# mhnazeri/PMoE

Measured on AMD Instinct MI355X. Metric: samples/sec fwd+bwd, 256x256 RGB 4-expert PMoE, higher is better.
Workload: dtype bf16; 1 GPU; 4-expert MoE (PMoE experts), 256x256x3 x4 frames, batch 64/GPU, fwd+moe_loss+bwd, dropout 0.3; global_batch=64, parallelism=dp1

## Files before the change

### pmoe_amd/csrc/conv_wgrad.hip

```cpp
#include "conv_common.h"
#include <stdlib.h>
#include "kernels.h"

template <typename T> struct WgradCfg;
template <> struct WgradCfg<bf16> { static constexpr int WCO = 2, WCI = 2, WK = 2, NW = 8; };
template <> struct WgradCfg<float> { static constexpr int WCO = 1, WCI = 1, WK = 4, NW = 4; };

typedef __attribute__((address_space(3))) s16x4 lds_s16x4;

__device__ __forceinline__ s16x4 tr_read(const char* p) {
    return __builtin_amdgcn_ds_read_tr16_b64_v4i16((lds_s16x4*)(p));
}

template <typename T, int TAPS, int MAXV>
__global__ void __launch_bounds__(WgradCfg<T>::NW * 64) conv_wgrad_kernel(const WgradArgs a) {
    constexpr int NTHR = WgradCfg<T>::NW * 64;
    constexpr int LOG_RB = 7, RB = 128;
    constexpr int VE = 16 / (int)sizeof(T);
    constexpr int CKW = RB / (int)sizeof(T);
    constexpr int WCI = WgradCfg<T>::WCI, WK = WgradCfg<T>::WK;
    constexpr int KS = TAPS == 9 ? 3 : 1;
    constexpr int MAXDY = 256 * 8 / NTHR;
    extern __shared__ __attribute__((aligned(16))) char smem[];

// ... 91 lines not shown
                int pA[2], ppB[2];
#pragma unroll
                for (int tt = 0; tt < 2; ++tt) {
                    const int p = p0 + 8 * (g >> 1) + 4 * tt + q;
                    pA[tt] = p;
                    const int mx = p & (TW - 1), my = (p >> lTW) & (TH - 1), pn = p >> (lTW + lTH);
                    ppB[tt] = (pn * PH + my * S) * PW + mx * S;
                }
                const int ca = (co_sub * 32 + cblk) * 2, cb = (ci_sub * 32 + cblk) * 2;
                bf16x8 fa;
#pragma unroll
                for (int tt = 0; tt < 2; ++tt) {
                    const s16x4 r = tr_read(dyt + pA[tt] * RS + ca);
                    const bf16x4 rb = __builtin_bit_cast(bf16x4, r);
#pragma unroll
                    for (int i = 0; i < 4; ++i) fa[4 * tt + i] = rb[i];
                }
                const char* bB[2] = {patch + ppB[0] * RS + cb, patch + ppB[1] * RS + cb};
#pragma unroll
                for (int tap = 0; tap < TAPS; ++tap) {
                    const int tapoff = ((tap / KS) * PW + (tap % KS)) * RS;
                    bf16x8 fb;
#pragma unroll
                    for (int tt = 0; tt < 2; ++tt) {
                        const s16x4 r = tr_read(bB[tt] + tapoff);
                        const bf16x4 rb = __builtin_bit_cast(bf16x4, r);
#pragma unroll
                        for (int i = 0; i < 4; ++i) fb[4 * tt + i] = rb[i];
                    }
                    acc[tap] = __builtin_amdgcn_mfma_f32_32x32x16_bf16(fa, fb, acc[tap], 0, 0, 0);
                }
            } else {
#pragma unroll
                for (int m = 0; m < 8; ++m) {
                    const int p = p0 + 2 * m + h;
                    const int mx = p & (TW - 1), my = (p >> lTW) & (TH - 1), pn = p >> (lTW + lTH);
                    const int ppb = (pn * PH + my * S) * PW + mx * S;
                    const float av = *reinterpret_cast<const float*>(dyt + p * RS + (l31 << 2));
#pragma unroll
                    for (int tap = 0; tap < TAPS; ++tap) {
                        const int pp = ppb + (tap / KS) * PW + (tap % KS);
                        const float bv = *reinterpret_cast<const float*>(patch + pp * RS + (l31 << 2));
                        acc[tap] = __builtin_amdgcn_mfma_f32_32x32x2f32(av, bv, acc[tap], 0, 0, 0);
                    }
                }
            }
        }
    }

    constexpr int TPR = TAPS == 9 ? 3 : 1;
    constexpr int TILE_WAVES = WCO * WCI;
    float* red = reinterpret_cast<float*>(smem);
    const int tw = wave % TILE_WAVES;
    const int cin = ci0 + ci_sub * 32 + l31;
    const size_t slab = a.per_image ? (size_t)e * a.ipe + split
                                    : (size_t)split * gridDim.z + e;
    float* dst = (a.per_image || nsplit == 1) ? a.dw : a.part;
#pragma unroll
    for (int t0 = 0; t0 < TAPS; t0 += TPR) {
        __syncthreads();
        if (k_sub > 0) {
#pragma unroll
            for (int tp = 0; tp < TPR; ++tp)
#pragma unroll
                for (int r = 0; r < 16; ++r)
                    red[((((k_sub - 1) * TPR + tp) * TILE_WAVES + tw) * 16 + r) * 64 + lane] = acc[t0 + tp][r];
        }
        __syncthreads();
        if (k_sub == 0) {
#pragma unroll
            for (int tp = 0; tp < TPR; ++tp) {
                float* base = dst + ((slab * TAPS + t0 + tp) * a.CoutP) * a.CinP;
#pragma unroll
                for (int r = 0; r < 16; ++r) {
                    float v = acc[t0 + tp][r];
#pragma unroll
                    for (int k = 1; k < WK; ++k) v += red[((((k - 1) * TPR + tp) * TILE_WAVES + tw) * 16 + r) * 64 + lane];
                    const int cout = co0 + co_sub * 32 + (r & 3) + 8 * (r >> 2) + 4 * h;
                    base[(size_t)cout * a.CinP + cin] = v;
                }
            }
        }
    }
}

template <int PIN, int WCI = 2, bool PAIRS = false, int REQ = 0>
__global__ void __launch_bounds__(512) conv_wgrad_dma_kernel(const WgradArgs a, const int magic_pw, const int magic_ph) {
    constexpr int TAPS = 9, RS = 128, CKW = 64;
    static_assert(!PAIRS || WCI == 1, "tap pairs: the narrow wave layout only");
    static_assert(REQ == 0 || (WCI == 2 && !PAIRS && PIN == 1), "precomputed requests: the 2 x 2 x 2 wave layout only");
    constexpr int WCO = 2, WK = 8 / (WCI * WCO);
    typedef __attribute__((address_space(3))) void lds_void;
    extern __shared__ __attribute__((aligned(16))) char smem[];

    const int tid = threadIdx.x, lane = tid & 63;
    const int wave = __builtin_amdgcn_readfirstlane(tid >> 6);
    const int l31 = lane & 31, h = lane >> 5;
    const int ci_sub = wave % WCI, co_sub = (wave / WCI) % WCO, k_sub = wave / (WCI * WCO);

    const int e = blockIdx.z;
    const int n_ci_blk = (a.Cin + CKW - 1) / CKW;
    const int npairs = n_ci_blk * ((a.Cout + CKW - 1) / CKW);
    const unsigned flat = xcd_remap(blockIdx.x, gridDim.x);
    const int nsplit = (int)(gridDim.x / npairs);
    const int pair = (int)(flat % npairs), split = (int)(flat / npairs);
    const int cob = pair / n_ci_blk, cib = pair % n_ci_blk;
    const int co0 = cob * CKW, ci0 = cib * CKW;

    const int lTW = a.lTW, lTH = a.lTH;
    const int TW = 1 << lTW, TH = 1 << lTH;
    const int PW = TW + 2, PH = TH + 2;
    const int NPIX = a.TN * PH * PW;
    const int NPIECE = (NPIX + 7) >> 3;
    const int BMP = a.TN << (lTW + lTH);
    const int XB = NPIECE << 10;
    const int pair_bytes = (BMP << 7) + XB;
    const int my_pieces = (NPIECE - wave + 7) >> 3;

    f32x16 acc[TAPS];
#pragma unroll
    for (int t = 0; t < TAPS; ++t)
#pragma unroll
        for (int k = 0; k < 16; ++k) acc[t][k] = 0.f;

    const int mbpe = a.n_groups * a.tiles_y * a.tiles_x;
    const int mb_begin = split * a.mb_per_wg;
    int mb_end = mb_begin + a.mb_per_wg;
    if (mb_end > mbpe) mb_end = mbpe;

    const bf16* xb = (const bf16*)a.x + (a.x_shared ? (size_t)0 : (size_t)e * a.ipe * a.H * a.W * a.x_ld) + a.x_coff + ci0;
    const bf16* dyb = (const bf16*)a.dy + (size_t)e * a.ipe * a.Ho * a.Wo * a.dy_ld + a.dy_coff + co0;
    const __amdgpu_buffer_rsrc_t rs_x = __builtin_amdgcn_make_buffer_rsrc(
        (void*)xb, (short)0, (int)(((long long)a.ipe * a.H * a.W * a.x_ld - a.x_coff - ci0) * 2), 0x00020000);
    const __amdgpu_buffer_rsrc_t rs_dy = __builtin_amdgcn_make_buffer_rsrc(
        (void*)dyb, (short)0, (int)(((long long)a.ipe * a.Ho * a.Wo * a.dy_ld - a.dy_coff - co0) * 2), 0x00020000);
    constexpr int OOB = 0x7ff80000;

    auto issue = [&](int mbi, int buf) {
        int t = mbi;
        const int px_t = t % a.tiles_x; t /= a.tiles_x;
        const int py_t = t % a.tiles_y; t /= a.tiles_y;
        const int n0 = t * a.TN;
        const int oy0 = py_t * TH, ox0 = px_t * TW;
        char* base = smem + buf * pair_bytes;
#pragma unroll
        for (int i = 0; i < 4; ++i) {
            const int p = ((wave + 8 * i) << 3) + (lane >> 3);
            const int mx = p & (TW - 1), my = (p >> lTW) & (TH - 1), pn = p >> (lTW + lTH);
            const int n = n0 + pn, oy = oy0 + my, ox = ox0 + mx;
            const int j = (lane & 7) ^ (((p >> 1) & 1) << 2);
            const bool ok = n < a.ipe && oy < a.Ho && ox < a.Wo && co0 + j * 8 < a.Cout;
            const int voff = ok ? ((((n * a.Ho + oy) * a.Wo + ox) * a.dy_ld) << 1) + (j << 4) : OOB;
            __builtin_amdgcn_raw_ptr_buffer_load_lds(rs_dy, (lds_void*)(base + ((wave + 8 * i) << 10)), 16, voff, 0, 0, 0);
        }
#pragma unroll
        for (int i = 0; i < 6; ++i) {
            if (i < my_pieces) {
                const int pp = ((wave + 8 * i) << 3) + (lane >> 3);
                const int rowq = (pp * magic_pw) >> 16, px = pp - rowq * PW;
                const int pn = (rowq * magic_ph) >> 16, prow = rowq - pn * PH;
                const int n = n0 + pn, Y = oy0 - a.pad + prow, X = ox0 - a.pad + px;
                const int j = (lane & 7) ^ (((px >> 1) & 1) << 2);
                const bool ok = pp < NPIX && n < a.ipe && (unsigned)Y < (unsigned)a.H && (unsigned)X < (unsigned)a.W &&
                                ci0 + j * 8 < a.Cin;
                const int voff = ok ? ((((n * a.H + Y) * a.W + X) * a.x_ld) << 1) + (j << 4) : OOB;
                __builtin_amdgcn_raw_ptr_buffer_load_lds(rs_x, (lds_void*)(base + (BMP << 7) + ((wave + 8 * i) << 10)), 16,
// ... 688 lines not shown
    const int pipe_unset = INT_MIN, pipe_sw = sw("PMOE_WGRAD_PIPE", pipe_unset);
    const bool narrow = a.Cin <= 32 && sw("PMOE_WGRAD_NARROW", 1);
    const bool v2 = !narrow && sw("PMOE_WGRAD_V2", 1) && pipe_sw == pipe_unset && (a.lTW == 4 || a.lTW == 5) && a.ipe <= 511;
    p->kind = v2 ? WGRAD_DMA2 : WGRAD_DMA;
    p->code = narrow ? 7109 : v2 ? 7309 : 7009;
    p->grid = dim3(p->nsplit * tiles, 1, p->E); p->block = dim3(512);
    p->smem = sm < 49152 ? 49152 : sm;
    const int pipe = pipe_sw == pipe_unset ? 1 : pipe_sw;
    p->pin = 1; p->wci = narrow ? 1 : 2;
    if (v2) {
#ifdef PMOE_STAMP
    } else if (pipe == 2 || pipe == 3) {
        p->pin = pipe; p->wci = 2;
#endif
    } else if (narrow) {
        p->pairs = a.Cin <= 16;
        if (p->smem < (size_t)3 * 3 * 2 * 4096) p->smem = (size_t)3 * 3 * 2 * 4096;
    } else if (pipe == 0) {
        p->pin = 0;
    } else {
        const int req = a.ipe > 511 ? 0 : sw("PMOE_WGRAD_REQ", 1);
        p->req = req == 1 || req == 2 ? req : 0;
    }
    return true;
}

template <typename T> constexpr int wgrad_fold_waves = (WgradCfg<T>::WK - 1) * WgradCfg<T>::WCO * WgradCfg<T>::WCI;

int wgrad_select(const WgradArgs& a0, int dtype, const WgradBn& bn, WgradPlan* p) {
    *p = WgradPlan{};
    p->a = a0;
    WgradArgs& a = p->a;
    auto done = [p](int code) { return p->code = code; };
    if (bn.fused) return done(wgrad_bnbwd_plan(dtype, bn.z_ld, p));
    if (dtype != PMOE_DT_BF16 && dtype != PMOE_DT_F32) return done(PMOE_ERR_ARG);
    const int esz = p->esz = dtype == PMOE_DT_BF16 ? 2 : 4;
    const int CKW = 128 / esz, VEh = 16 / esz, NW = esz == 2 ? WgradCfg<bf16>::NW : WgradCfg<float>::NW;
    const int M1 = 48 / NW, M2 = 80 / NW;
    if (a.Cin % VEh || a.Cout % VEh || a.CinP < a.Cin || a.CoutP < a.Cout) return done(PMOE_ERR_ARG);
    if (a.CinP != (a.Cin + CKW - 1) / CKW * CKW || a.CoutP != (a.Cout + CKW - 1) / CKW * CKW) return done(PMOE_ERR_ARG);
    if ((a.ks != 1 && a.ks != 3) || (a.stride != 1 && a.stride != 2) || a.N % a.ipe) return done(PMOE_ERR_ARG);
    p->E = a.N / a.ipe; p->taps = a.ks * a.ks;
    const int lstride = a.ks == 1 ? 1 : a.stride;
    int lBM = 8, PW, PH, NPIX, need;
    size_t smem;
    for (;; --lBM) {
        if (lBM < 6) return done(PMOE_ERR_UNSUPPORTED);
        set_tile(a, pixel_tile(a.Ho, a.Wo, a.ipe, lBM, 5));
        PW = patch_extent(a.lTW, a.ks, lstride); PH = patch_extent(a.lTH, a.ks, lstride);
        NPIX = a.TN * PH * PW;
        need = (NPIX * 8 + NW * 64 - 1) / (NW * 64);
        smem = ((size_t)(1 << lBM) + NPIX) * 192;
        if (need <= M2 && smem <= 150 * 1024) break;
    }
    const int mbpe = a.n_groups * a.tiles_y * a.tiles_x;
    const int tiles = ((a.Cout + CKW - 1) / CKW) * ((a.Cin + CKW - 1) / CKW);
    const int target = 256;
    int want = (target + tiles * p->E - 1) / (tiles * p->E);
    if (want < 1) want = 1;
    if (want > mbpe) want = mbpe;
    a.mb_per_wg = (mbpe + want - 1) / want;
    if (a.per_image) {
        if (a.TN != 1) return done(PMOE_ERR_UNSUPPORTED);
        a.mb_per_wg = a.tiles_y * a.tiles_x;
    }
    a.slice_fastest = 0;
    p->nsplit = (mbpe + a.mb_per_wg - 1) / a.mb_per_wg;
    p->ws_floats = (a.per_image || p->nsplit == 1) ? 0 : (long long)p->nsplit * p->E * p->taps * a.CoutP * a.CinP;
    if (esz == 2 && lBM == 8 && wgrad_dma_plan(NPIX, PW, PH, tiles, p)) return p->code;
    p->kind = WGRAD_TILE;
    p->maxv = need <= M1 ? M1 : M2;
    p->grid = dim3(p->nsplit * tiles, 1, p->E); p->block = dim3(NW * 64);
    const size_t fold = (size_t)(esz == 2 ? wgrad_fold_waves<bf16> : wgrad_fold_waves<float>) * (p->taps == 9 ? 3 : 1) * 4096;
    p->smem = smem < fold ? fold : smem;
    return p->code = 6000 + p->taps * 100 + p->maxv;
}

template <auto KERNEL, typename... Args> static int wgrad_go(const WgradPlan& p, hipStream_t st, const Args&... args) {
    return launch<KERNEL>(p.grid, p.block, p.smem, st, p.a, args...);
}

template <typename T> static int wgrad_tile_launch(const WgradPlan& p, hipStream_t st) {
    constexpr int M1 = 48 / WgradCfg<T>::NW, M2 = 80 / WgradCfg<T>::NW;
    if (p.maxv == M1) return p.taps == 9 ? wgrad_go<conv_wgrad_kernel<T, 9, M1>>(p, st) : wgrad_go<conv_wgrad_kernel<T, 1, M1>>(p, st);
    return p.taps == 9 ? wgrad_go<conv_wgrad_kernel<T, 9, M2>>(p, st) : wgrad_go<conv_wgrad_kernel<T, 1, M2>>(p, st);
}

static int wgrad_dma_launch(const WgradPlan& p, hipStream_t st) {
    switch (p.pin) {
    case 0: return wgrad_go<conv_wgrad_dma_kernel<0>>(p, st, p.mpw, p.mph);
#ifdef PMOE_STAMP
    case 2: return wgrad_go<conv_wgrad_dma_kernel<2>>(p, st, p.mpw, p.mph);
    case 3: return wgrad_go<conv_wgrad_dma_kernel<3>>(p, st, p.mpw, p.mph);
#endif
    }
    if (p.wci == 1 && p.pairs) return wgrad_go<conv_wgrad_dma_kernel<1, 1, true>>(p, st, p.mpw, p.mph);
    if (p.wci == 1) return wgrad_go<conv_wgrad_dma_kernel<1, 1>>(p, st, p.mpw, p.mph);
    if (p.req == 2) return wgrad_go<conv_wgrad_dma_kernel<1, 2, false, 2>>(p, st, p.mpw, p.mph);
    if (p.req == 1) return wgrad_go<conv_wgrad_dma_kernel<1, 2, false, 1>>(p, st, p.mpw, p.mph);
    return wgrad_go<conv_wgrad_dma_kernel<1>>(p, st, p.mpw, p.mph);
}

static int wgrad_dma2_launch(const WgradPlan& p, hipStream_t st) {
    if (p.a.lTW == 5) return wgrad_go<conv_wgrad_dma2_kernel<5>>(p, st, p.mpw, p.mph);
    return wgrad_go<conv_wgrad_dma2_kernel<4>>(p, st, p.mpw, p.mph);
}

static int conv_wgrad_bnbwd_launch(const WgradPlan& p, const WgradBn& bn, hipStream_t st) {
    if (!bn.z || !bn.coef || !bn.c1 || !bn.c2 || !p.a.x || !p.a.dy || !p.a.dw) return PMOE_ERR_ARG;
    return wgrad_go<conv_wgrad_bnbwd_kernel>(p, st, BnBwdFuse{bn.z, bn.coef, bn.c1, bn.c2, bn.z_ld, p.a.Cout});
}

int conv_wgrad_launch(const WgradArgs& a, int dtype, const WgradBn& bn, hipStream_t st) {
    WgradPlan p;
    if (wgrad_select(a, dtype, bn, &p) < 0) return p.code;
    if (p.ws_floats > 0 && (!a.part || a.part_floats < p.ws_floats)) return PMOE_ERR_ARG;
    const int rc = p.kind == WGRAD_BNBWD ? conv_wgrad_bnbwd_launch(p, bn, st)
                 : p.kind == WGRAD_DMA2 ? wgrad_dma2_launch(p, st)
                 : p.kind == WGRAD_DMA ? wgrad_dma_launch(p, st)
                 : p.esz == 2 ? wgrad_tile_launch<bf16>(p, st) : wgrad_tile_launch<float>(p, st);
    return rc ? rc : wgrad_finish(p, st);
}

int conv_wgrad_fold(const WgradArgs& a, int dtype, const WgradBn& bn, hipStream_t st) {
    WgradPlan p;
    if (wgrad_select(a, dtype, bn, &p) < 0) return p.code;
    if (p.ws_floats > 0 && (!a.part || a.part_floats < p.ws_floats)) return PMOE_ERR_ARG;
    return wgrad_finish(p, st, true);
}

int conv_wgrad_plan(const WgradArgs& a, int dtype, const WgradBn& bn) {
    WgradPlan p;
    return wgrad_select(a, dtype, bn, &p);
}

long long conv_wgrad_ws_floats(const WgradArgs& a, int dtype, const WgradBn& bn) {
    WgradPlan p;
    return wgrad_select(a, dtype, bn, &p) < 0 ? p.code : p.ws_floats;
}
```

### pmoe_amd/csrc/conv_c16.hip

```cpp
#include "common.h"
#include "kernels.h"

namespace {

typedef unsigned v4u __attribute__((ext_vector_type(4)));
typedef float f32x2 __attribute__((ext_vector_type(2)));

__global__ void __launch_bounds__(256, 2) conv3x3_c16_kernel(ConvArgs a, int tiles_x, int tiles_per_expert, int wgs_per_expert,
                                                            unsigned in_bytes, unsigned out_bytes) {
    __shared__ v4i wl[18][64];
    __shared__ v4i tbuf[4][256];
    __shared__ float red[4][8][2][64];
    const int tid = threadIdx.x, lane = tid & 63;
    const int wave = __builtin_amdgcn_readfirstlane(tid >> 6);
    const int e = blockIdx.y, wg = blockIdx.x;
    {
        const bf16* w = reinterpret_cast<const bf16*>(a.w) + (size_t)e * a.CoutP * 9 * 16;
        for (int idx = tid; idx < 18 * 64; idx += 256) {
            const int l = idx & 63, mtap = idx >> 6, mt = mtap / 9, tap = mtap - mt * 9;
            const int m = l & 31, kh = l >> 5;
            const int aa = m >> 3, hh = (m >> 2) & 1, b = m & 3;
            const int cout = 16 * (2 * mt + (aa >> 1)) + 8 * hh + 4 * (aa & 1) + b;
            wl[mtap][l] = ldg16(w + ((size_t)cout * 9 + tap) * 16 + kh * 8);
        }
    }
    __syncthreads();
    const size_t in_img0 = a.in_shared ? 0 : (size_t)e * a.ipe, out_img0 = (size_t)e * a.ipe;
    const __amdgpu_buffer_rsrc_t rs_in = __builtin_amdgcn_make_buffer_rsrc(
        (void*)(reinterpret_cast<const bf16*>(a.in) + in_img0 * a.H * a.W * a.in_ld + a.in_coff - a.in_ld), (short)0,
        (int)(in_bytes + (unsigned)a.in_ld * 2u), 0x00020000);
    const __amdgpu_buffer_rsrc_t rs_out = __builtin_amdgcn_make_buffer_rsrc(
        (void*)(reinterpret_cast<bf16*>(a.out) + out_img0 * a.H * a.W * a.out_ld + a.out_coff), (short)0, (int)out_bytes, 0x00020000);
    constexpr unsigned OOB = 0xfffffff0u;
    const int px_l = lane & 31, kh = lane >> 5;
    const unsigned ld2 = (unsigned)a.in_ld * 2u, old2 = (unsigned)a.out_ld * 2u;
    const unsigned vin = (unsigned)(px_l + 1) * ld2 + (unsigned)kh * 16u;
    unsigned vout[4];
#pragma unroll
    for (int i = 0; i < 4; ++i) vout[i] = (unsigned)(i * 8 + (lane >> 3)) * old2 + (unsigned)(lane & 7) * 16u;
    const bool chunk_ok = (lane & 7) * 8 < a.Cout;
    const int t0 = (int)((long long)tiles_per_expert * wg / wgs_per_expert);
    const int t1 = (int)((long long)tiles_per_expert * (wg + 1) / wgs_per_expert);
    f32x2 s1[4], s2[4];
#pragma unroll
    for (int j = 0; j < 4; ++j) s1[j] = s2[j] = f32x2{0.f, 0.f};

    struct Pos { int xt, y, img; };
    auto advance = [&](Pos& p) {
        p.xt += 4;
        while (p.xt >= tiles_x) { p.xt -= tiles_x; if (++p.y == a.H) { p.y = 0; ++p.img; } }
    };
    auto load_tile = [&](const Pos& p, v4u (&raw)[9], bool live) {
        const unsigned row0 = ((unsigned)(p.img * a.H + p.y) * (unsigned)a.W + (unsigned)p.xt * 32u) * ld2;
        const int px = p.xt * 32 + px_l;
        unsigned vq[3];
        vq[0] = live && px >= 1 && px - 1 < a.W ? vin - ld2 : OOB;
        vq[1] = live && px < a.W ? vin : OOB;
        vq[2] = live && px + 1 < a.W ? vin + ld2 : OOB;
#pragma unroll
        for (int r = 0; r < 3; ++r) {
            const int yy = p.y + r - 1;
            const bool row_ok = live && (unsigned)yy < (unsigned)a.H;
            const unsigned soff = row_ok ? row0 + (unsigned)(r - 1) * (unsigned)a.W * ld2 : 0u;
#pragma unroll
            for (int q = 0; q < 3; ++q)
                raw[r * 3 + q] = __builtin_amdgcn_raw_buffer_load_b128(rs_in, (int)(row_ok ? vq[q] : OOB), (int)soff, 0);
        }
    };
    auto process = [&](const Pos& pc, const v4u (&cur)[9]) {
        f32x16 acc[2];
#pragma unroll
        for (int mt = 0; mt < 2; ++mt)
#pragma unroll
            for (int i = 0; i < 16; ++i) acc[mt][i] = 0.f;
#pragma unroll
        for (int tap = 0; tap < 9; ++tap)
#pragma unroll
            for (int mt = 0; mt < 2; ++mt)
                acc[mt] = __builtin_amdgcn_mfma_f32_32x32x16_bf16(__builtin_bit_cast(bf16x8, wl[mt * 9 + tap][lane]),
                                                                  __builtin_bit_cast(bf16x8, cur[tap]), acc[mt], 0, 0, 0);
#pragma unroll
        for (int g = 0; g < 4; ++g) {
            float v[8];
#pragma unroll
            for (int i = 0; i < 8; ++i) v[i] = acc[g >> 1][8 * (g & 1) + i];
            tbuf[wave][px_l * 8 + ((2 * g + kh) ^ (px_l & 7))] = pack16<bf16>(v);
        }
        const unsigned osoff = ((unsigned)(pc.img * a.H + pc.y) * (unsigned)a.W + (unsigned)pc.xt * 32u) * old2;
#pragma unroll
        for (int i = 0; i < 4; ++i) {
            const int p = i * 8 + (lane >> 3), c = lane & 7;
            const v4i v = tbuf[wave][p * 8 + (c ^ (p & 7))];
            const bool ok = pc.xt * 32 + p < a.W;
            __builtin_amdgcn_raw_buffer_store_b128(__builtin_bit_cast(v4u, v), rs_out, (int)(ok && chunk_ok ? vout[i] : OOB), (int)osoff, 0);
            if (a.stats && ok) {
                float rr[8];
                unpack16<bf16>(v, rr);
#pragma unroll
                for (int q = 0; q < 4; ++q) {
                    const f32x2 r2 = f32x2{rr[2 * q], rr[2 * q + 1]};
                    s1[q] += r2;
                    s2[q] = __builtin_elementwise_fma(r2, r2, s2[q]);
                }
            }
        }
    };
    Pos pl, pc;
    {
        const int t = t0 + wave;
        pl.xt = t % tiles_x;
        const int r = t / tiles_x;
        pl.y = r % a.H;
        pl.img = r / a.H;
        pc = pl;
    }
    v4u b0[9], b1[9], b2[9];
    int tl = t0 + wave, t = tl;
    auto fetch = [&](v4u (&buf)[9]) {
        load_tile(pl, buf, tl < t1);
        advance(pl);
        tl += 4;
    };
    fetch(b0);
    fetch(b1);
    while (t < t1) {
        fetch(b2);
        process(pc, b0); advance(pc); t += 4;
        if (t >= t1) break;
        fetch(b0);
        process(pc, b1); advance(pc); t += 4;
        if (t >= t1) break;
        fetch(b1);
        process(pc, b2); advance(pc); t += 4;
    }
    if (!a.stats) return;
#pragma unroll
    for (int q = 0; q < 8; ++q) {
        red[wave][lane >> 3][0][(lane & 7) * 8 + q] = s1[q >> 1][q & 1];
        red[wave][lane >> 3][1][(lane & 7) * 8 + q] = s2[q >> 1][q & 1];
    }
    __syncthreads();
    if (tid < 128) {
        const int which = tid >> 6, c = tid & 63;
        float s = 0.f;
        for (int w = 0; w < 4; ++w)
            for (int pg = 0; pg < 8; ++pg) s += red[w][pg][which][c];
        a.stats[(((size_t)e * wgs_per_expert + wg) * 2 + which) * a.CoutP + c] = s;
    }
}

}

bool conv_c16_plan(const ConvArgs& a, int dtype, ConvLaunch* l) {
    if (!sw("PMOE_CONV_C16", 1)) return false;
    if (dtype != PMOE_DT_BF16 || a.w_fp8 || a.ks != 3 || a.stride != 1 || a.pad != 1 || a.dilate) return false;
    if (a.Cin != 16 || a.CoutP != 64 || a.Cout % 8 || a.Cout > 64) return false;
    if (a.bias || a.act != PMOE_ACT_NONE || a.res_mode != PMOE_RES_NONE || a.drop_p > 0.f) return false;
    if (a.N % a.ipe || a.Ho != a.H || a.Wo != a.W) return false;
    if (a.in_ld % 8 || a.in_coff % 8 || a.out_ld % 8 || a.out_coff % 8) return false;
    if ((long long)a.ipe * a.H * a.W * (a.in_ld > a.out_ld ? a.in_ld : a.out_ld) * 2 >= 0xfff00000ll) return false;
    const int E = a.N / a.ipe, tx = (a.W + 31) / 32;
    const long long tpe = (long long)a.ipe * a.H * tx;
    if (tpe > 0x7fffffffll || tpe < 64) return false;
    int wpe = 512 / E;
    if (wpe < 1) wpe = 1;
    if (wpe > tpe / 16) wpe = (int)(tpe / 16);
    if (wpe < 1) wpe = 1;
    l->kind = CONV_C16; l->code = 1316; l->a = a;
    l->wpe = wpe; l->tiles_x = tx; l->tpe = (int)tpe; l->mblocks = E * wpe;
    return true;
}

int conv_c16_launch(const ConvLaunch& l, hipStream_t st) {
    const ConvArgs& a = l.a;
    const long long in_b = (long long)a.ipe * a.H * a.W * a.in_ld * 2 - (long long)a.in_coff * 2;
    const long long out_b = (long long)a.ipe * a.H * a.W * a.out_ld * 2 - (long long)a.out_coff * 2;
    return launch<conv3x3_c16_kernel, 0>(dim3(l.wpe, a.N / a.ipe), dim3(256), 0, st, a, l.tiles_x, l.tpe, l.wpe, (unsigned)in_b, (unsigned)out_b);
}
```

### pmoe_amd/csrc/elementwise.hip

```cpp
#include "common.h"

template <typename T, int MODE>
__global__ void __launch_bounds__(256) colstats_kernel(const T* __restrict__ x, const T* __restrict__ dy,
                                                      const T* __restrict__ y, const float* __restrict__ mean,
                                                      const float* __restrict__ invstd, const float* __restrict__ scale,
                                                      const float* __restrict__ shift, long long rpe, int C, int ld,
                                                      int coff, int relu, float* __restrict__ part, int nparts,
                                                      float* __restrict__ shiftc, T* __restrict__ gmask) {
    constexpr int VE = 16 / (int)sizeof(T);
    const int CV = C / VE, RL = 256 / CV;
    const int tid = threadIdx.x, cv = tid % CV, rl = tid / CV;
    const int e = blockIdx.y, pi = blockIdx.x;
    const long long rpp = (rpe + nparts - 1) / nparts;
    long long r0 = (long long)pi * rpp, r1 = r0 + rpp;
    if (r1 > rpe) r1 = rpe;
    float s1[VE], s2[VE], mu[VE], is[VE], sc[VE], sh[VE];
    const bool remask = MODE && relu && !y;
#pragma unroll
    for (int i = 0; i < VE; ++i) {
        s1[i] = s2[i] = 0.f;
        mu[i] = MODE ? mean[e * C + cv * VE + i] : 0.f;
        is[i] = MODE ? invstd[e * C + cv * VE + i] : 0.f;
        sc[i] = remask ? scale[e * C + cv * VE + i] : 0.f;
        sh[i] = remask ? shift[e * C + cv * VE + i] : 0.f;
// ... 360 lines not shown
        const int yy = (int)(t % H);
        const int n = (int)(t / H);
        float g[VE];
#pragma unroll
        for (int k = 0; k < VE; ++k) g[k] = 0.f;
        const int oy_lo = yy >> 1, oy_hi = (yy + 1) >> 1, ox_lo = xx >> 1, ox_hi = (xx + 1) >> 1;
        for (int oy = oy_lo; oy <= oy_hi; ++oy)
            for (int ox = ox_lo; ox <= ox_hi; ++ox) {
                if (oy >= Ho || ox >= Wo) continue;
                const int r = yy - (2 * oy - 1), q = xx - (2 * ox - 1);
                const size_t off = ((((size_t)n * Ho + oy) * Wo + ox) * CV + cv) * VE;
                float d[VE];
                unpack16<T>(ldg16(dy + off), d);
                const int tap = r * 3 + q;
#pragma unroll
                for (int k = 0; k < VE; ++k)
                    if (am[off + k] == tap) g[k] += d[k];
            }
        stg16(dx + (size_t)i * VE, pack16<T>(g));
    }
}

template <typename T>
__global__ void __launch_bounds__(256) gap_partial_kernel(const T* __restrict__ a, const T* __restrict__ b,
                                                         float* __restrict__ part, long long HW, int C, int nparts,
                                                         int b_ipe) {
    constexpr int VE = 16 / (int)sizeof(T);
    const int CV = C / VE, RL = 256 / CV;
    const int tid = threadIdx.x, cv = tid % CV, rl = tid / CV;
    const int n = blockIdx.y, pi = blockIdx.x;
    const long long rpp = (HW + nparts - 1) / nparts;
    long long r0 = (long long)pi * rpp, r1 = r0 + rpp;
    if (r1 > HW) r1 = HW;
    const int nb = b_ipe > 0 ? n % b_ipe : n;
    float s[VE];
#pragma unroll
    for (int i = 0; i < VE; ++i) s[i] = 0.f;
    if (rl >= RL) r0 = r1;
    for (long long r = r0 + rl; r < r1; r += RL) {
        float av[VE];
        unpack16<T>(ldg16(a + ((size_t)n * HW + r) * C + cv * VE), av);
        if (b) {
            float bv[VE];
            unpack16<T>(ldg16(b + ((size_t)nb * HW + r) * C + cv * VE), bv);
#pragma unroll
            for (int i = 0; i < VE; ++i) s[i] += av[i] * bv[i];
        } else {
#pragma unroll
            for (int i = 0; i < VE; ++i) s[i] += av[i];
        }
    }
    __shared__ float red[256 * 8];
#pragma unroll
    for (int i = 0; i < VE; ++i)
        if (rl < RL) red[rl * C + cv * VE + i] = s[i];
    __syncthreads();
    for (int c = tid; c < C; c += 256) {
        float t = 0.f;
        for (int k = 0; k < RL; ++k) t += red[k * C + c];
        part[((size_t)n * nparts + pi) * C + c] = t;
    }
}

template <typename T>
__global__ void __launch_bounds__(256) bn_apply_gap_kernel(const T* __restrict__ x, T* __restrict__ y,
                                                          const float* __restrict__ scale, const float* __restrict__ shift,
                                                          const float* __restrict__ mean, float* __restrict__ part,
                                                          long long HW, int C, int nparts, int ipe, int relu) {
    constexpr int VE = 16 / (int)sizeof(T);
    const int CV = C / VE, RL = 256 / CV;
    const int tid = threadIdx.x, cv = tid % CV, rl = tid / CV;
    const int n = blockIdx.y, pi = blockIdx.x, e = n / ipe;
    const long long rpp = (HW + nparts - 1) / nparts;
    long long r0 = (long long)pi * rpp, r1 = r0 + rpp;
    if (r1 > HW) r1 = HW;
    float s[VE], sc[VE], sh[VE], mu[VE];
#pragma unroll
    for (int i = 0; i < VE; ++i) {
        s[i] = 0.f;
        const int c = e * C + (rl < RL ? cv : 0) * VE + i;
        sc[i] = scale[c]; sh[i] = shift[c]; mu[i] = mean[c];
    }
    if (rl >= RL) r0 = r1;
    for (long long r = r0 + rl; r < r1; r += RL) {
        const size_t off = ((size_t)n * HW + r) * C + cv * VE;
        float xv[VE];
        unpack16<T>(ldg16(x + off), xv);
#pragma unroll
        for (int i = 0; i < VE; ++i) {
            xv[i] = (xv[i] - mu[i]) * sc[i] + sh[i];
            if (relu) xv[i] = fmaxf(xv[i], 0.f);
        }
        const v4i pk = pack16<T>(xv);
        stg16(y + off, pk);
        float yv[VE];
        unpack16<T>(pk, yv);
#pragma unroll
        for (int i = 0; i < VE; ++i) s[i] += yv[i];
    }
    __shared__ float red[256 * 8];
#pragma unroll
    for (int i = 0; i < VE; ++i)
        if (rl < RL) red[rl * C + cv * VE + i] = s[i];
    __syncthreads();
    for (int c = tid; c < C; c += 256) {
        float t = 0.f;
        for (int k = 0; k < RL; ++k) t += red[k * C + c];
        part[((size_t)n * nparts + pi) * C + c] = t;
    }
}

template <typename T>
__global__ void __launch_bounds__(256) gap_finish_kernel(const float* __restrict__ part, T* __restrict__ out, int N,
                                                        int C, int nparts, float inv_hw, int out_ld, int out_coff) {
    const long long total = (long long)N * C;
    for (long long i = (long long)blockIdx.x * 256 + threadIdx.x; i < total; i += (long long)gridDim.x * 256) {
        const int c = (int)(i % C), n = (int)(i / C);
        float s = 0.f;
        for (int k = 0; k < nparts; ++k) s += part[((size_t)n * nparts + k) * C + c];
        out[(size_t)n * out_ld + out_coff + c] = from_f32<T>(s * inv_hw);
    }
}

template <typename T>
__global__ void __launch_bounds__(256) gap_bwd_kernel(const T* __restrict__ g, T* __restrict__ dx, long long HW, int C,
                                                     int g_ld, int g_coff, float inv_hw) {
    constexpr int VE = 16 / (int)sizeof(T);
    const int CV = C / VE;
    const int n = blockIdx.y;
    const long long nvec = HW * CV;
    for (long long i = (long long)blockIdx.x * 256 + threadIdx.x; i < nvec; i += (long long)gridDim.x * 256) {
        const int cv = (int)(i % CV);
        float v[VE];
        unpack16<T>(ldg16(g + (size_t)n * g_ld + g_coff + cv * VE), v);
#pragma unroll
        for (int k = 0; k < VE; ++k) v[k] *= inv_hw;
        stg16(dx + ((size_t)n * HW) * C + (size_t)i * VE, pack16<T>(v));
    }
}

__global__ void __launch_bounds__(256) eca_gate_kernel(const float* __restrict__ part, int nparts, float inv_hw,
                                                      const float* const* w, int k, float* __restrict__ gate,
                                                      float* __restrict__ gapmean, int ipe, int in_ipe, int C,
                                                      int creal) {
    const int n = blockIdx.x, e = n / ipe;
    const int ni = in_ipe > 0 ? n % ipe : n;
    __shared__ float gm[1024];
    for (int c = threadIdx.x; c < C; c += 256) {
        float s = 0.f;
        for (int i = 0; i < nparts; ++i) s += part[((size_t)ni * nparts + i) * C + c];
        gm[c] = c < creal ? s * inv_hw : 0.f;
    }
    __syncthreads();
    const float* we = w[e];
    const int pad = k / 2;
    for (int c = threadIdx.x; c < C; c += 256) {
        float z = 0.f;
        for (int j = 0; j < k; ++j) {
            const int cc = c + j - pad;
            if (cc >= 0 && cc < creal) z += we[j] * gm[cc];
        }
        gate[(size_t)n * C + c] = c < creal ? 1.f / (1.f + expf(-z)) : 0.f;
        gapmean[(size_t)n * C + c] = gm[c];
    }
}

template <typename T>
__global__ void __launch_bounds__(256) eca_scale_kernel(const T* __restrict__ x, const float* __restrict__ gate,
                                                       T* __restrict__ y, long long HW, int C, int x_ipe) {
    constexpr int VE = 16 / (int)sizeof(T);
    const int CV = C / VE;
    const int n = blockIdx.y;
    const int nx = x_ipe > 0 ? n % x_ipe : n;
    const long long nvec = HW * CV;
    for (long long i = (long long)blockIdx.x * 256 + threadIdx.x; i < nvec; i += (long long)gridDim.x * 256) {
        const int cv = (int)(i % CV);
        float v[VE];
        unpack16<T>(ldg16(x + (size_t)nx * HW * C + (size_t)i * VE), v);
#pragma unroll
        for (int k = 0; k < VE; ++k) v[k] *= gate[(size_t)n * C + cv * VE + k];
        stg16(y + (size_t)n * HW * C + (size_t)i * VE, pack16<T>(v));
// ... 376 lines not shown
```

Baseline: 1838 samples/s.

## Add warp-specialized stride-2 3x3 bf16 weight-gradient kernel with loader waves

Adds a dedicated kernel for bf16 stride-2 3x3 weight gradients. Four waves act as producers that prefetch dy and input patches into registers and commit them to LDS, while the other four waves run MFMA over all nine taps with a register ring of transposed LDS reads. The aim is to overlap global loads with matrix math and to avoid the generic tile kernel's cross-wave K reduction. The trade-offs are that only half the waves issue MFMA and that correctness depends on the new patch geometry and guard logic.

```diff
diff --git a/pmoe_amd/csrc/conv_wgrad.hip b/pmoe_amd/csrc/conv_wgrad.hip
--- a/pmoe_amd/csrc/conv_wgrad.hip
+++ b/pmoe_amd/csrc/conv_wgrad.hip
@@ -197,6 +197,182 @@
             }
         }
     }
+}
+
+template <int MAXV>
+__device__ __forceinline__ void conv_wgrad_s2_split_body(const WgradArgs& a) {
+    constexpr int TAPS = 9, KS = 3, S = 2, RS = 192, XRS = 192, CKW = 64, LOG_RB = 7, VE = 8;
+    constexpr int NLD = 256;
+    constexpr int MAXDY = 256 * 8 / NLD, AHEAD = 5, RINGB = 6;
+    extern __shared__ __attribute__((aligned(16))) char smem[];
+    const int tid = threadIdx.x, lane = tid & 63;
+    const int wave = __builtin_amdgcn_readfirstlane(tid >> 6);
+    const int l31 = lane & 31, h = lane >> 5;
+
+    const int e = blockIdx.z;
+    const int n_ci_blk = (a.Cin + CKW - 1) / CKW;
+    const int npairs = n_ci_blk * ((a.Cout + CKW - 1) / CKW);
+    const unsigned flat = xcd_remap(blockIdx.x, gridDim.x);
+    const int nsplit = (int)(gridDim.x / npairs);
+    const int pair = (int)(flat % npairs), split = (int)(flat / npairs);
+    const int cob = pair / n_ci_blk, cib = pair % n_ci_blk;
+    const int co0 = cob * CKW, ci0 = cib * CKW;
+
+    const int lTW = a.lTW, lTH = a.lTH;
+    const int TW = 1 << lTW, TH = 1 << lTH;
+    const int PW = (TW - 1) * S + KS, PH = (TH - 1) * S + KS;
+    const int NPIX = a.TN * PH * PW;
+    const int BMP = a.TN << (lTW + lTH);
+    const int mbpe = a.n_groups * a.tiles_y * a.tiles_x;
+    const int mb_begin = split * a.mb_per_wg;
+    int mb_end = mb_begin + a.mb_per_wg;
+    if (mb_end > mbpe) mb_end = mbpe;
+
+    char* dyt = smem;
+    char* patch = smem + BMP * RS;
+
+    if (wave >= 4) {
+        const int lt = tid - NLD;
+        const bf16* x = (const bf16*)a.x;
+        const bf16* dy = (const bf16*)a.dy;
+        PatchStage<bf16, LOG_RB, NLD, 2 * MAXV> xs;
+        v4i dyv[MAXDY];
+        const int dyj = lt & 7;
+        const bool dy_cok = co0 + dyj * VE < a.Cout;
+        constexpr int GUARD = (1 << 9) | (1 << 19) | (1 << 29);
+        int drel[MAXDY], dgeo[MAXDY], xrel[2 * MAXV], xgeo[2 * MAXV];
+#pragma unroll
+        for (int u = 0; u < MAXDY; ++u) {
+            const int p = (lt >> 3) + u * (NLD / 8);
+            const int mx = p & (TW - 1), my = (p >> lTW) & (TH - 1), pn = p >> (lTW + lTH);
+            drel[u] = ((pn * a.Ho + my) * a.Wo + mx) * a.dy_ld;
+            dgeo[u] = (p < BMP && dy_cok ? (pn << 20) | (my << 10) | mx : (511 << 20)) | GUARD;
+        }
+        const bool x_cok = ci0 + dyj * VE < a.Cin;
+#pragma unroll
+        for (int u = 0; u < 2 * MAXV; ++u) {
+            const int pp = (lt >> 3) + u * (NLD / 8);
+            const int row = pp / PW, ix = pp - row * PW;
+            const int pn = row / PH, iy = row - pn * PH;
+            xrel[u] = ((pn * a.H + iy) * a.W + ix) * a.x_ld;
+            xgeo[u] = (pp < NPIX && x_cok ? (pn << 20) | (iy << 10) | ix : (511 << 20)) | GUARD;
+        }
+        auto imin = [](int u, int v) { return u < v ? u : v; };
+        auto issue = [&](int mbi) {
+            int t = mbi;
+            const int px = t % a.tiles_x; t /= a.tiles_x;
+            const int py = t % a.tiles_y; t /= a.tiles_y;
+            const int n0 = e * a.ipe + t * a.TN;
+            const int nmax = imin((e + 1) * a.ipe - n0, 511) - 1;
+            const int oy0 = py * TH, ox0 = px * TW, Y0 = oy0 * S - a.pad, X0 = ox0 * S - a.pad;
+            const bf16* dyb = dy + (((size_t)n0 * a.Ho + oy0) * a.Wo + ox0) * a.dy_ld + a.dy_coff + co0 + dyj * VE;
+            const int dkk = (((nmax << 20) | ((imin(TH, a.Ho - oy0) - 1) << 10) | (imin(TW, a.Wo - ox0) - 1)) | GUARD) + GUARD;
+#pragma unroll
+            for (int u = 0; u < MAXDY; ++u) {
+                dyv[u] = v4i{0, 0, 0, 0};
+                if (((dkk - dgeo[u]) & GUARD) == GUARD) dyv[u] = ldg16(dyb + drel[u]);
+            }
+            const long long xoff = (((long long)(a.x_shared ? n0 - e * a.ipe : n0) * a.H + Y0) * a.W + X0) * a.x_ld + a.x_coff + ci0 + dyj * VE;
+            const int xlo = ((Y0 < 0 ? -Y0 : 0) << 10) | (X0 < 0 ? -X0 : 0);
+            const int xkk = (((nmax << 20) | ((imin(PH, a.H - Y0) - 1) << 10) | (imin(PW, a.W - X0) - 1)) | GUARD) + GUARD;
+#pragma unroll
+            for (int u = 0; u < 2 * MAXV; ++u) {
+                xs.v[u] = v4i{0, 0, 0, 0};
+                if (((xgeo[u] - xlo) & (xkk - xgeo[u]) & GUARD) == GUARD) xs.v[u] = ldg16(x + (xoff + xrel[u]));
+            }
+        };
+        if (mb_begin < mb_end) issue(mb_begin);
+        for (int mbi = mb_begin; mbi < mb_end; ++mbi) {
+            __syncthreads();
+#pragma unroll
+            for (int u = 0; u < MAXDY; ++u) {
+                const int p = (lt >> 3) + u * (NLD / 8);
+                if (p < BMP) *reinterpret_cast<v4i*>(dyt + lds_chunk_off<LOG_RB, 2>(p, dyj)) = dyv[u];
+            }
+            xs.template commit<2>(patch, NPIX, lt);
+            __syncthreads();
+            if (mbi + 1 < mb_end) issue(mbi + 1);
+        }
+        return;
+    }
+
+    const int co_sub = wave >> 1, ci_sub = wave & 1;
+    f32x16 acc[TAPS];
+#pragma unroll
+    for (int t = 0; t < TAPS; ++t)
+#pragma unroll
+        for (int k = 0; k < 16; ++k) acc[t][k] = 0.f;
+    const int g = lane >> 4, q = (lane >> 2) & 3, pc = lane & 3;
+    const int cblk = 16 * (g & 1) + 4 * pc;
+    const int ca = (co_sub * 32 + cblk) * 2, cb = (ci_sub * 32 + cblk) * 2;
+    int la[2];
+#pragma unroll
+    for (int tt = 0; tt < 2; ++tt) la[tt] = (8 * (g >> 1) + 4 * tt + q) * RS + ca;
+    const int rowoff = PW * XRS;
+    const int nkb = BMP >> 4;
+    auto xbase = [&](int kb, int tt) {
+        const int p = (kb << 4) + 8 * (g >> 1) + 4 * tt + q;
+        const int mx = p & (TW - 1), my = (p >> lTW) & (TH - 1), pn = p >> (lTW + lTH);
+        return patch + ((pn * PH + my * S) * PW + mx * S) * XRS + cb;
+    };
+    auto frag8 = [](const s16x4& u0, const s16x4& u1) {
+        const bf16x4 u = __builtin_bit_cast(bf16x4, u0), v = __builtin_bit_cast(bf16x4, u1);
+        return bf16x8{u[0], u[1], u[2], u[3], v[0], v[1], v[2], v[3]};
+    };
+    s16x4 fa_[2][2], fb_[RINGB][2];
+
+    for (int mbi = mb_begin; mbi < mb_end; ++mbi) {
+        __syncthreads();
+        __syncthreads();
+        {
+            const char* b0[2] = {xbase(0, 0), xbase(0, 1)};
+#pragma unroll
+            for (int tt = 0; tt < 2; ++tt) fa_[0][tt] = tr_read(dyt + la[tt]);
+#pragma unroll
+            for (int u = 0; u < AHEAD; ++u)
+#pragma unroll
+                for (int tt = 0; tt < 2; ++tt) fb_[u % RINGB][tt] = tr_read(b0[tt] + (u / 3) * rowoff + (u % 3) * XRS);
+        }
+#pragma unroll 1
+        for (int kb0 = 0; kb0 < nkb; kb0 += 2) {
+            const int kb2 = kb0 + 2 < nkb ? kb0 + 2 : 0;
+            const char* br[3][2] = {{xbase(kb0, 0), xbase(kb0, 1)}, {xbase(kb0 + 1, 0), xbase(kb0 + 1, 1)}, {xbase(kb2, 0), xbase(kb2, 1)}};
+#pragma unroll
+            for (int v = 0; v < 18; ++v) {
+                const int kbl = v / 9, tap = v % 9;
+                acc[tap] = __builtin_amdgcn_mfma_f32_32x32x16_bf16(frag8(fa_[kbl][0], fa_[kbl][1]),
+                                                                   frag8(fb_[v % RINGB][0], fb_[v % RINGB][1]), acc[tap], 0, 0, 0);
+                const int w = v + AHEAD, wk = w / 9, wt = w % 9;
+                if (kb0 + wk < nkb) {
+#pragma unroll
+                    for (int tt = 0; tt < 2; ++tt) fb_[w % RINGB][tt] = tr_read(br[wk][tt] + (wt / 3) * rowoff + (wt % 3) * XRS);
+                }
+                if (tap == 3 && kb0 + kbl + 1 < nkb) {
+#pragma unroll
+                    for (int tt = 0; tt < 2; ++tt) fa_[(kbl + 1) & 1][tt] = tr_read(dyt + (kb0 + kbl + 1) * (16 * RS) + la[tt]);
+                }
+                __builtin_amdgcn_sched_barrier(0);
+            }
+        }
+    }
+
+    const int cin = ci0 + ci_sub * 32 + l31;
+    const size_t slab = a.per_image ? (size_t)e * a.ipe + split : (size_t)split * gridDim.z + e;
+    float* dst = (a.per_image || nsplit == 1) ? a.dw : a.part;
+#pragma unroll
+    for (int tap = 0; tap < TAPS; ++tap) {
+        float* base = dst + ((slab * TAPS + tap) * a.CoutP) * a.CinP;
+#pragma unroll
+        for (int r = 0; r < 16; ++r) {
+            const int cout = co0 + co_sub * 32 + (r & 3) + 8 * (r >> 2) + 4 * h;
+            base[(size_t)cout * a.CinP + cin] = acc[tap][r];
+        }
+    }
+}
+
+template <int MAXV>
+__global__ void __launch_bounds__(512) conv_wgrad_s2_kernel(const WgradArgs a) {
+    conv_wgrad_s2_split_body<MAXV>(a);
 }
 
 template <int PIN, int WCI = 2, bool PAIRS = false, int REQ = 0>
@@ -1051,6 +1227,10 @@
 
 template <typename T> static int wgrad_tile_launch(const WgradPlan& p, hipStream_t st) {
     constexpr int M1 = 48 / WgradCfg<T>::NW, M2 = 80 / WgradCfg<T>::NW;
+    if constexpr (sizeof(T) == 2) {
+        if (p.taps == 9 && p.a.stride == 2)
+            return p.maxv == M1 ? wgrad_go<conv_wgrad_s2_kernel<M1>>(p, st) : wgrad_go<conv_wgrad_s2_kernel<M2>>(p, st);
+    }
     if (p.maxv == M1) return p.taps == 9 ? wgrad_go<conv_wgrad_kernel<T, 9, M1>>(p, st) : wgrad_go<conv_wgrad_kernel<T, 1, M1>>(p, st);
     return p.taps == 9 ? wgrad_go<conv_wgrad_kernel<T, 9, M2>>(p, st) : wgrad_go<conv_wgrad_kernel<T, 1, M2>>(p, st);
 }
```

Result: no change. 1826 samples/s (-0.6%).

## Load conv3x3 c16 center column plus halo and share neighbors via bpermute

Applied to the files above, without the earlier changes.

The 3x3 Cin=16 conv kernel now loads only the center pixel for each of three rows plus one halo load per lane, instead of nine shifted buffer loads per tile. Left and right neighbors come from ds_bpermute lane shuffles, with tile edges taken from the halo. The pipeline becomes a configurable N-buffer ring with dummy OOB stores that balance vmcnt, and optional timing stamps sit behind macros. Separately, the GAP fused normalize kernel unrolls its row loop by four so loads are issued ahead of compute. The trade is fewer global loads for extra LDS-path permute instructions and more complex edge handling.

```diff
diff --git a/pmoe_amd/csrc/conv_c16.hip b/pmoe_amd/csrc/conv_c16.hip
--- a/pmoe_amd/csrc/conv_c16.hip
+++ b/pmoe_amd/csrc/conv_c16.hip
@@ -5,6 +5,15 @@
 
 typedef unsigned v4u __attribute__((ext_vector_type(4)));
 typedef float f32x2 __attribute__((ext_vector_type(2)));
+
+#ifndef C16_NB
+#define C16_NB 3
+#endif
+#ifdef PMOE_STAMP
+#define CLAP(i) { __builtin_amdgcn_sched_barrier(0); const unsigned long long st_t = __builtin_amdgcn_s_memtime(); st_acc[i] += (unsigned)(st_t - st_prev); st_prev = st_t; __builtin_amdgcn_sched_barrier(0); }
+#else
+#define CLAP(i)
+#endif
 
 __global__ void __launch_bounds__(256, 2) conv3x3_c16_kernel(ConvArgs a, int tiles_x, int tiles_per_expert, int wgs_per_expert,
                                                             unsigned in_bytes, unsigned out_bytes) {
@@ -14,6 +23,12 @@
     const int tid = threadIdx.x, lane = tid & 63;
     const int wave = __builtin_amdgcn_readfirstlane(tid >> 6);
     const int e = blockIdx.y, wg = blockIdx.x;
+#ifdef PMOE_STAMP
+    unsigned long long st_prev = __builtin_amdgcn_s_memtime();
+    const unsigned long long st_r0 = __builtin_amdgcn_s_memrealtime();
+    unsigned st_acc[4] = {0, 0, 0, 0};
+    int ntile = 0;
+#endif
     {
         const bf16* w = reinterpret_cast<const bf16*>(a.w) + (size_t)e * a.CoutP * 9 * 16;
         for (int idx = tid; idx < 18 * 64; idx += 256) {
@@ -35,10 +50,19 @@
     const int px_l = lane & 31, kh = lane >> 5;
     const unsigned ld2 = (unsigned)a.in_ld * 2u, old2 = (unsigned)a.out_ld * 2u;
     const unsigned vin = (unsigned)(px_l + 1) * ld2 + (unsigned)kh * 16u;
+    const int h_r = lane >> 2, h_s = (lane >> 1) & 1;
+    const unsigned hoff = (unsigned)(h_r - 1) * (unsigned)a.W * ld2 + (h_s ? 33u : 0u) * ld2 + (unsigned)(lane & 1) * 16u;
+    const int idx_l = ((lane - 1) & 63) * 4, idx_r = ((lane + 1) & 63) * 4;
+    const int idx_h = ((px_l == 31 ? 2 : 0) + kh) * 4;
+    const bool first_px = px_l == 0, last_px = px_l == 31;
     unsigned vout[4];
 #pragma unroll
     for (int i = 0; i < 4; ++i) vout[i] = (unsigned)(i * 8 + (lane >> 3)) * old2 + (unsigned)(lane & 7) * 16u;
+#ifdef C16_NOSTORE
+    const bool chunk_ok = false;
+#else
     const bool chunk_ok = (lane & 7) * 8 < a.Cout;
+#endif
     const int t0 = (int)((long long)tiles_per_expert * wg / wgs_per_expert);
     const int t1 = (int)((long long)tiles_per_expert * (wg + 1) / wgs_per_expert);
     f32x2 s1[4], s2[4];
@@ -48,37 +72,53 @@
     struct Pos { int xt, y, img; };
     auto advance = [&](Pos& p) {
         p.xt += 4;
-        while (p.xt >= tiles_x) { p.xt -= tiles_x; if (++p.y == a.H) { p.y = 0; ++p.img; } }
-    };
-    auto load_tile = [&](const Pos& p, v4u (&raw)[9], bool live) {
+#pragma unroll
+        for (int k = 0; k < 4; ++k)
+            if (p.xt >= tiles_x) { p.xt -= tiles_x; if (++p.y == a.H) { p.y = 0; ++p.img; } }
+    };
+    auto load_tile = [&](const Pos& p, v4u (&raw)[4], bool live) {
+#ifdef C16_NOLOAD
+        live = false;
+#endif
         const unsigned row0 = ((unsigned)(p.img * a.H + p.y) * (unsigned)a.W + (unsigned)p.xt * 32u) * ld2;
-        const int px = p.xt * 32 + px_l;
-        unsigned vq[3];
-        vq[0] = live && px >= 1 && px - 1 < a.W ? vin - ld2 : OOB;
-        vq[1] = live && px < a.W ? vin : OOB;
-        vq[2] = live && px + 1 < a.W ? vin + ld2 : OOB;
+        const unsigned vc = live && p.xt * 32 + px_l < a.W ? vin : OOB;
+        const bool up_ok = live && p.y > 0, dn_ok = live && p.y + 1 < a.H;
 #pragma unroll
         for (int r = 0; r < 3; ++r) {
-            const int yy = p.y + r - 1;
-            const bool row_ok = live && (unsigned)yy < (unsigned)a.H;
+            const bool row_ok = r == 0 ? up_ok : r == 2 ? dn_ok : live;
             const unsigned soff = row_ok ? row0 + (unsigned)(r - 1) * (unsigned)a.W * ld2 : 0u;
+            raw[r] = __builtin_amdgcn_raw_buffer_load_b128(rs_in, (int)(row_ok ? vc : OOB), (int)soff, 0);
+        }
+        const bool h_row = h_r == 0 ? up_ok : h_r == 2 ? dn_ok : live && h_r == 1;
+        const bool h_col = h_s ? p.xt * 32 + 32 < a.W : p.xt > 0;
+        raw[3] = __builtin_amdgcn_raw_buffer_load_b128(rs_in, (int)(h_row && h_col ? row0 + hoff : OOB), 0, 0);
+    };
+    auto mfma_tile = [&](const v4u (&raw)[4], f32x16 (&acc)[2]) {
+#pragma unroll
+        for (int mt = 0; mt < 2; ++mt)
+#pragma unroll
+            for (int i = 0; i < 16; ++i) acc[mt][i] = 0.f;
+#pragma unroll
+        for (int r = 0; r < 3; ++r) {
+            v4u col[3];
+            col[1] = raw[r];
+#pragma unroll
+            for (int d = 0; d < 4; ++d) {
+                const unsigned hv = (unsigned)__builtin_amdgcn_ds_bpermute(idx_h + 16 * r, (int)raw[3][d]);
+                const unsigned lv = (unsigned)__builtin_amdgcn_ds_bpermute(idx_l, (int)raw[r][d]);
+                const unsigned rv = (unsigned)__builtin_amdgcn_ds_bpermute(idx_r, (int)raw[r][d]);
+                col[0][d] = first_px ? hv : lv;
+                col[2][d] = last_px ? hv : rv;
+            }
 #pragma unroll
             for (int q = 0; q < 3; ++q)
-                raw[r * 3 + q] = __builtin_amdgcn_raw_buffer_load_b128(rs_in, (int)(row_ok ? vq[q] : OOB), (int)soff, 0);
-        }
-    };
-    auto process = [&](const Pos& pc, const v4u (&cur)[9]) {
-        f32x16 acc[2];
-#pragma unroll
-        for (int mt = 0; mt < 2; ++mt)
-#pragma unroll
-            for (int i = 0; i < 16; ++i) acc[mt][i] = 0.f;
-#pragma unroll
-        for (int tap = 0; tap < 9; ++tap)
-#pragma unroll
-            for (int mt = 0; mt < 2; ++mt)
-                acc[mt] = __builtin_amdgcn_mfma_f32_32x32x16_bf16(__builtin_bit_cast(bf16x8, wl[mt * 9 + tap][lane]),
-                                                                  __builtin_bit_cast(bf16x8, cur[tap]), acc[mt], 0, 0, 0);
+#pragma unroll
+                for (int mt = 0; mt < 2; ++mt)
+                    acc[mt] = __builtin_amdgcn_mfma_f32_32x32x16_bf16(__builtin_bit_cast(bf16x8, wl[mt * 9 + r * 3 + q][lane]),
+                                                                      __builtin_bit_cast(bf16x8, col[q]), acc[mt], 0, 0, 0);
+        }
+    };
+    auto stage_tile = [&](const f32x16 (&acc)[2]) {
 #pragma unroll
         for (int g = 0; g < 4; ++g) {
             float v[8];
@@ -86,12 +126,14 @@
             for (int i = 0; i < 8; ++i) v[i] = acc[g >> 1][8 * (g & 1) + i];
             tbuf[wave][px_l * 8 + ((2 * g + kh) ^ (px_l & 7))] = pack16<bf16>(v);
         }
+    };
+    auto drain_tile = [&](const Pos& pc, bool live) {
         const unsigned osoff = ((unsigned)(pc.img * a.H + pc.y) * (unsigned)a.W + (unsigned)pc.xt * 32u) * old2;
 #pragma unroll
         for (int i = 0; i < 4; ++i) {
             const int p = i * 8 + (lane >> 3), c = lane & 7;
             const v4i v = tbuf[wave][p * 8 + (c ^ (p & 7))];
-            const bool ok = pc.xt * 32 + p < a.W;
+            const bool ok = live && pc.xt * 32 + p < a.W;
             __builtin_amdgcn_raw_buffer_store_b128(__builtin_bit_cast(v4u, v), rs_out, (int)(ok && chunk_ok ? vout[i] : OOB), (int)osoff, 0);
             if (a.stats && ok) {
                 float rr[8];
@@ -114,26 +156,53 @@
         pl.img = r / a.H;
         pc = pl;
     }
-    v4u b0[9], b1[9], b2[9];
     int tl = t0 + wave, t = tl;
-    auto fetch = [&](v4u (&buf)[9]) {
+    auto fetch = [&](v4u (&buf)[4]) {
         load_tile(pl, buf, tl < t1);
         advance(pl);
         tl += 4;
     };
-    fetch(b0);
-    fetch(b1);
+    auto step = [&](const v4u (&cur)[4]) {
+        f32x16 acc[2];
+#ifdef PMOE_STAMP
+        CLAP(3)
+        asm volatile("s_waitcnt vmcnt(%0)" ::"n"((C16_NB - 1) * 8) : "memory");
+        CLAP(0)
+        ntile += t < t1;
+#endif
+        mfma_tile(cur, acc);
+        stage_tile(acc);
+        CLAP(1)
+        drain_tile(pc, t < t1);
+        CLAP(2)
+        advance(pc);
+        t += 4;
+    };
+    v4u buf[C16_NB][4];
+#pragma unroll
+    for (int i = 0; i < C16_NB - 1; ++i) {
+        fetch(buf[i]);
+#pragma unroll
+        for (int j = 0; j < 4; ++j)
+            __builtin_amdgcn_raw_buffer_store_b128(v4u{0u, 0u, 0u, 0u}, rs_out, (int)(OOB - 16u * (unsigned)(4 * i + j)), 0, 0);
+    }
     while (t < t1) {
-        fetch(b2);
-        process(pc, b0); advance(pc); t += 4;
-        if (t >= t1) break;
-        fetch(b0);
-        process(pc, b1); advance(pc); t += 4;
-        if (t >= t1) break;
-        fetch(b1);
-        process(pc, b2); advance(pc); t += 4;
+#pragma unroll
+        for (int i = 0; i < C16_NB; ++i) {
+            fetch(buf[(i + C16_NB - 1) % C16_NB]);
+            step(buf[i]);
+        }
     }
     if (!a.stats) return;
+#ifdef PMOE_STAMP
+    if (lane == 0) {
+        float* o = a.stats + ((size_t)e * wgs_per_expert + wg) * 2 * a.CoutP + wave * 8;
+        for (int i = 0; i < 4; ++i) o[i] = (float)st_acc[i];
+        o[4] = (float)(unsigned)(__builtin_amdgcn_s_memrealtime() - st_r0);
+        o[5] = (float)ntile;
+    }
+    return;
+#endif
 #pragma unroll
     for (int q = 0; q < 8; ++q) {
         red[wave][lane >> 3][0][(lane & 7) * 8 + q] = s1[q >> 1][q & 1];
diff --git a/pmoe_amd/csrc/elementwise.hip b/pmoe_amd/csrc/elementwise.hip
--- a/pmoe_amd/csrc/elementwise.hip
+++ b/pmoe_amd/csrc/elementwise.hip
@@ -466,10 +466,9 @@
         sc[i] = scale[c]; sh[i] = shift[c]; mu[i] = mean[c];
     }
     if (rl >= RL) r0 = r1;
-    for (long long r = r0 + rl; r < r1; r += RL) {
-        const size_t off = ((size_t)n * HW + r) * C + cv * VE;
+    auto row = [&](size_t off, const v4i& raw) {
         float xv[VE];
-        unpack16<T>(ldg16(x + off), xv);
+        unpack16<T>(raw, xv);
 #pragma unroll
         for (int i = 0; i < VE; ++i) {
             xv[i] = (xv[i] - mu[i]) * sc[i] + sh[i];
@@ -481,6 +480,21 @@
         unpack16<T>(pk, yv);
 #pragma unroll
         for (int i = 0; i < VE; ++i) s[i] += yv[i];
+    };
+    constexpr int GAP_UNROLL = 4;
+    const size_t base = (size_t)n * HW * C + cv * VE, rstep = (size_t)RL * C;
+    long long r = r0 + rl;
+    for (; r + (GAP_UNROLL - 1) * RL < r1; r += GAP_UNROLL * RL) {
+        const size_t off = base + (size_t)r * C;
+        v4i raw[GAP_UNROLL];
+#pragma unroll
+        for (int u = 0; u < GAP_UNROLL; ++u) raw[u] = ldg16(x + off + u * rstep);
+#pragma unroll
+        for (int u = 0; u < GAP_UNROLL; ++u) row(off + u * rstep, raw[u]);
+    }
+    for (; r < r1; r += RL) {
+        const size_t off = base + (size_t)r * C;
+        row(off, ldg16(x + off));
     }
     __shared__ float red[256 * 8];
 #pragma unroll
```

New measurement: 1907 samples/s before, 1930 samples/s after, median of 6. No clear change (+1.2%).
